# bschrag620/PyRad

Measured on NVIDIA B200. Metric: line-gridpoint evals/s, higher is better.
Workload: dtype f32

## Files before the change

### pyrad_b200/csrc/k2_line_sum.cuh

```cuda
#pragma once
#include "common.cuh"
#include "k3_stream.cuh"

namespace prb {

__device__ __forceinline__ float rcp_approx(float x) {
    float r;
    asm("rcp.approx.ftz.f32 %0, %1;" : "=f"(r) : "f"(x));
    return r;
}
__device__ __forceinline__ float ex2_approx(float x) {
    float r;
    asm("ex2.approx.ftz.f32 %0, %1;" : "=f"(r) : "f"(x));
    return r;
}

__device__ __forceinline__ void tma_bulk_s2g(void *dst, const void *src, uint32_t bytes) {
    asm volatile("cp.async.bulk.global.shared::cta.bulk_group [%0], [%1], %2;" ::"l"(dst), "r"(smem_u32(src)), "r"(bytes)
                 : "memory");
}
__device__ __forceinline__ void consumer_barrier() {
    asm volatile("bar.sync 1, %0;" ::"n"(K2_CONSUMERS * 32) : "memory");
}

__device__ __forceinline__ int warp_lower_bound(const int32_t *__restrict__ idx, int lo, int hi, long long key) {
    const int lane = threadIdx.x & 31;
    while (hi > lo) {
        const int span = hi - lo;
        const int step = (span + 31) >> 5;
        int pos = lo + (lane + 1) * step - 1;
        pos = pos < hi - 1 ? pos : hi - 1;
        const bool less = (long long)__ldg(idx + pos) < key;
        const unsigned m = __ballot_sync(0xffffffffu, less);
        const int c = __popc(m);
        int nlo = lo, nhi = hi;
        if (c > 0) { int p = lo + c * step - 1; p = p < hi - 1 ? p : hi - 1; nlo = p + 1; }
        if (c < 32) { int p = lo + (c + 1) * step - 1; p = p < hi - 1 ? p : hi - 1; nhi = p; }
        lo = nlo;
        hi = nhi;
    }
    return lo;
}

constexpr int K2_MAX_XSC = 8;
struct K2Layer {
    const float4 *recA;
    const float4 *recB;
    const float *recD;
    void *out;
    double inv_scale;
    int l_begin, l_end;
    int wm;
    int pad;
    double xsc_w[K2_MAX_XSC];
};

constexpr int K2_MAX_PEERS = 8;
constexpr int K2_MAX_DST = K2_MAX_PEERS + 1;
struct K2Fuse {
    int enabled;
    int n_dst;
    float neg_depth_log2e;
    float c2_over_t, c2_over_tsurf;
    long long n_total;
    double x0, dx, x_last;
    float *rad[K2_MAX_DST];
    float *trans[K2_MAX_DST];
};

struct K2Args {
    const K2Layer *layers;
    int n_layers;
    const int32_t *idx;
    long long i_begin;
    int n_chunk;
    int n_tiles;
    int tile_base;
    const int2 *tile_bounds;
    int variant;
    int out_mode;
    DevState *st;
    K2Fuse fuse;
    const double *far_lag;
    float far_delta[16];
    const double *far_lag2;
    float far_delta2[16];
    const double *xsc_sigma;
    long long xsc_ld;
    int n_xsc;
    int parts;
    double *part_sums;
    unsigned int *part_count;
};

__device__ __forceinline__ double k2_add_xsc(const K2Args &a, const K2Layer *L, int i, double v) {
    for (int t = 0; t < a.n_xsc; ++t)
        v = __dadd_rn(v, __dmul_rn(__ldg(a.xsc_sigma + (long long)t * a.xsc_ld + i), __ldg(&L->xsc_w[t])));
    return v;
}

constexpr int K2_FAR_NODES = 16;
constexpr int K2_FAR_RADIUS_SPANS = 1;
constexpr int K2_FAR_SUBGROUPS = 64 / K2_FAR_NODES;
constexpr int K2_FAR_FLUSH = 16;
#ifndef PRB_K2_FAR2_SPANS
#define PRB_K2_FAR2_SPANS 8
#endif
constexpr int K2_FAR2_SPANS = PRB_K2_FAR2_SPANS;
#ifndef PRB_K2_FAR2_ENABLE
#define PRB_K2_FAR2_ENABLE 1
#endif
constexpr bool K2_FAR2 = PRB_K2_FAR2_ENABLE != 0;
constexpr int K2_FAR2_MIN_DOMAINS = 4;
static_assert(K2_CONSUMERS % K2_FAR2_SPANS == 0, "a tile is a whole number of level-2 domains");

struct K2Desc {
    int tile0;
    int cnt;
    int flags;
    int layer;
    int part;
};
constexpr int K2_FIRST = 1, K2_LAST = 2, K2_END = 4;

struct K2Smem {
    float4 rA[K2_STAGES][K2_CHUNK];
    float4 rB[K2_STAGES][K2_CHUNK];
    float rD[K2_STAGES][K2_CHUNK];
    K2Desc desc[K2_STAGES];
    uint64_t full[K2_STAGES];
    uint64_t empty[K2_STAGES];
    double far2[2][K2_CONSUMERS][K2_FAR_NODES];
    double2 faracc[2][K2_CONSUMERS * 32];
    int part_last;
};

template <int P>
__host__ __device__ constexpr size_t K2_SMEM_BASE() {
    return ((sizeof(K2Smem) + (PRB_K2_ACC_SMEM ? sizeof(double) * P * K2_CONSUMERS * 32 : 0)) + 127) & ~size_t(127);
}
template <int P>
__host__ __device__ constexpr size_t K2_SMEM_BYTES(bool peer_staging) {
    return K2_SMEM_BASE<P>() + (peer_staging ? sizeof(float) * 2 * K2_CONSUMERS * 32 * P : 0);
}

template <int H>
struct Acc {
    float2 fi[H];
    float2 a32[H];
#if PRB_K2_ACC_SMEM
    double *a64;
    __device__ __forceinline__ double &acc(int p) { return a64[p * (K2_CONSUMERS * 32)]; }
#else
    double a64[2 * H];
    __device__ __forceinline__ double &acc(int p) { return a64[p]; }
#endif
    __device__ __forceinline__ void flush() {
#pragma unroll
        for (int j = 0; j < H; ++j) {
            acc(2 * j) += (double)a32[j].x;
            acc(2 * j + 1) += (double)a32[j].y;
            a32[j] = make_float2(0.f, 0.f);
        }
    }
};

__device__ __forceinline__ float2 splat(float v) { return make_float2(v, v); }
__device__ __forceinline__ float2 lo2(const float4 &v) { return make_float2(v.x, v.y); }
__device__ __forceinline__ float2 hi2(const float4 &v) { return make_float2(v.z, v.w); }

template <int H, bool MASKED>
__device__ __forceinline__ void triple_step(const float4 &a1, const float4 &a2, const float4 &a3, const float2 &B1,
                                            const float2 &B2, const float2 &B3, float wmf, Acc<H> &s) {
    const float2 nf1 = lo2(a1), nf2 = lo2(a2), nf3 = lo2(a3);
#pragma unroll
    for (int h = 0; h < H; ++h) {
        const float2 e1 = __fadd2_rn(s.fi[h], nf1);
        const float2 e2 = __fadd2_rn(s.fi[h], nf2);
        const float2 e3 = __fadd2_rn(s.fi[h], nf3);
        const float2 q1 = __ffma2_rn(e1, e1, B1);
        const float2 q2 = __ffma2_rn(e2, e2, B2);
        const float2 q3 = __ffma2_rn(e3, e3, B3);
        float2 A1 = hi2(a1), A2 = hi2(a2), A3 = hi2(a3);
        if (MASKED) {
            A1.x = fabsf(e1.x) <= wmf ? A1.x : 0.f;
            A1.y = fabsf(e1.y) <= wmf ? A1.y : 0.f;
            A2.x = fabsf(e2.x) <= wmf ? A2.x : 0.f;
            A2.y = fabsf(e2.y) <= wmf ? A2.y : 0.f;
            A3.x = fabsf(e3.x) <= wmf ? A3.x : 0.f;
            A3.y = fabsf(e3.y) <= wmf ? A3.y : 0.f;
        }
        const float2 p23 = __fmul2_rn(q2, q3);
        const float2 t = __ffma2_rn(A3, q2, __fmul2_rn(A2, q3));
        const float2 num = __ffma2_rn(q1, t, __fmul2_rn(A1, p23));
        const float2 den = __fmul2_rn(q1, p23);
        const float2 r = make_float2(rcp_approx(den.x), rcp_approx(den.y));
        s.a32[h] = __ffma2_rn(num, r, s.a32[h]);
    }
}

__device__ __forceinline__ float2 ldB(const float4 *sB, int j) { return *reinterpret_cast<const float2 *>(sB + j); }

template <int H, bool MASKED>
__device__ __forceinline__ void lorentz_paired(const float4 *sA, const float4 *sB, int js, int je, float wmf,
                                               Acc<H> &s) {
    const int n = je - js;
    if (n <= 0) return;
    int j = js;
    const int n6 = (n / 6) * 6;
    const int jq = js + n6;
    if (n6) {
        float4 xa1 = sA[j], xa2 = sA[j + 1], xa3 = sA[j + 2], ya1 = sA[j + 3], ya2 = sA[j + 4], ya3 = sA[j + 5];
        float2 xb1 = ldB(sB, j), xb2 = ldB(sB, j + 1), xb3 = ldB(sB, j + 2);
        float2 yb1 = ldB(sB, j + 3), yb2 = ldB(sB, j + 4), yb3 = ldB(sB, j + 5);
        int since = 0;
        for (j += 6; j < jq; j += 6) {
            triple_step<H, MASKED>(xa1, xa2, xa3, xb1, xb2, xb3, wmf, s);
            xa1 = sA[j]; xa2 = sA[j + 1]; xa3 = sA[j + 2];
            xb1 = ldB(sB, j); xb2 = ldB(sB, j + 1); xb3 = ldB(sB, j + 2);
            triple_step<H, MASKED>(ya1, ya2, ya3, yb1, yb2, yb3, wmf, s);
            ya1 = sA[j + 3]; ya2 = sA[j + 4]; ya3 = sA[j + 5];
            yb1 = ldB(sB, j + 3); yb2 = ldB(sB, j + 4); yb3 = ldB(sB, j + 5);
            if (++since == K2_FLUSH / 6) { s.flush(); since = 0; }
        }
        triple_step<H, MASKED>(xa1, xa2, xa3, xb1, xb2, xb3, wmf, s);
        triple_step<H, MASKED>(ya1, ya2, ya3, yb1, yb2, yb3, wmf, s);
    }
    for (j = jq; j < je; j += 3) {
        const float4 a1 = sA[j];
        const float2 B1 = ldB(sB, j);
        const float4 z = make_float4(a1.x, a1.y, 0.f, 0.f);
        const bool h2 = j + 1 < je, h3 = j + 2 < je;
        triple_step<H, MASKED>(a1, h2 ? sA[j + 1] : z, h3 ? sA[j + 2] : z, B1, h2 ? ldB(sB, j + 1) : B1,
                               h3 ? ldB(sB, j + 2) : B1, wmf, s);
    }
    s.flush();
}

#ifndef PRB_K2_GAUSS_PAIR_H
#define PRB_K2_GAUSS_PAIR_H 2
#endif
constexpr int K2_GAUSS_PAIR_H = PRB_K2_GAUSS_PAIR_H;

template <int H, bool MASKED>
__device__ __forceinline__ void gauss_pass(const float4 *sA, const float4 *sB, const float *sD, int js, int je,
                                           float wbf, float we1f, float wmf, Acc<H> &s) {
    int since = 0;
    for (int jb = js; jb < je; jb += 32) {
        const int jt = jb + (int)(threadIdx.x & 31);
        bool hit = false;
        if (jt < je) {
            const float dg = sD[jt];
            const float f = -sA[jt].x;
            hit = (dg >= 0.f) && (f + dg >= wbf) && (f - dg <= we1f);
        }
        unsigned int m = __ballot_sync(0xffffffffu, hit);
        auto one = [&](const float4 &b, float nf1) {
            const float2 nf = splat(nf1), C2 = splat(b.w);
#pragma unroll
            for (int h = 0; h < H; ++h) {
                const float2 e = __fadd2_rn(s.fi[h], nf);
                const float2 arg = __fmul2_rn(C2, __fmul2_rn(e, e));
                float2 g = splat(b.z);
                if (MASKED) {
                    g.x = fabsf(e.x) <= wmf ? b.z : 0.f;
                    g.y = fabsf(e.y) <= wmf ? b.z : 0.f;
                }
                s.a32[h] = __ffma2_rn(g, make_float2(ex2_approx(arg.x), ex2_approx(arg.y)), s.a32[h]);
            }
        };
        while (m) {
            const int j = jb + __ffs(m) - 1;
            m &= m - 1;
            if (H <= K2_GAUSS_PAIR_H && m) {
                const int j2 = jb + __ffs(m) - 1;
                m &= m - 1;
                const float4 b1 = sB[j], b2 = sB[j2];
                const float n1 = sA[j].x, n2 = sA[j2].x;
                const float2 nfa = splat(n1), nfb = splat(n2), Ca = splat(b1.w), Cb = splat(b2.w);
                float2 ta[H], tb[H], ga[H], gb[H];
#pragma unroll
                for (int h = 0; h < H; ++h) {
                    const float2 ea = __fadd2_rn(s.fi[h], nfa), eb = __fadd2_rn(s.fi[h], nfb);
                    const float2 xa = __fmul2_rn(Ca, __fmul2_rn(ea, ea)), xb = __fmul2_rn(Cb, __fmul2_rn(eb, eb));
                    ga[h] = splat(b1.z);
                    gb[h] = splat(b2.z);
                    if (MASKED) {
                        ga[h].x = fabsf(ea.x) <= wmf ? b1.z : 0.f;
                        ga[h].y = fabsf(ea.y) <= wmf ? b1.z : 0.f;
                        gb[h].x = fabsf(eb.x) <= wmf ? b2.z : 0.f;
                        gb[h].y = fabsf(eb.y) <= wmf ? b2.z : 0.f;
                    }
                    ta[h] = make_float2(ex2_approx(xa.x), ex2_approx(xa.y));
                    tb[h] = make_float2(ex2_approx(xb.x), ex2_approx(xb.y));
                }
#pragma unroll
                for (int h = 0; h < H; ++h) s.a32[h] = __ffma2_rn(gb[h], tb[h], __ffma2_rn(ga[h], ta[h], s.a32[h]));
                since += 2;
                if (since >= K2_FLUSH) { s.flush(); since = 0; }
                continue;
            }
            one(sB[j], sA[j].x);
            if (++since >= K2_FLUSH) { s.flush(); since = 0; }
        }
    }
    if (since) s.flush();
}

struct FarAcc {
    double v0, v1;
};
__device__ __forceinline__ float2 far_triple(const float4 &a1, const float4 &a2, const float4 &a3, const float2 &B1,
                                             const float2 &B2, const float2 &B3, const float2 &A1, const float2 &A2,
                                             const float2 &A3, const float2 &wb2, const float2 &del, const float2 &part) {
    const float2 e1 = __fadd2_rn(__fadd2_rn(wb2, lo2(a1)), del);
    const float2 e2 = __fadd2_rn(__fadd2_rn(wb2, lo2(a2)), del);
    const float2 e3 = __fadd2_rn(__fadd2_rn(wb2, lo2(a3)), del);
    const float2 q1 = __ffma2_rn(e1, e1, B1);
    const float2 q2 = __ffma2_rn(e2, e2, B2);
    const float2 q3 = __ffma2_rn(e3, e3, B3);
    const float2 p23 = __fmul2_rn(q2, q3);
    const float2 t = __ffma2_rn(A3, q2, __fmul2_rn(A2, q3));
    const float2 num = __ffma2_rn(q1, t, __fmul2_rn(A1, p23));
    const float2 den = __fmul2_rn(q1, p23);
    const float2 r = make_float2(rcp_approx(den.x), rcp_approx(den.y));
    return __ffma2_rn(num, r, part);
}
template <int G>
__device__ __forceinline__ void far_pass(const float4 *sA, const float4 *sB, int js, int je, float wbf, float2 del,
                                         double2 *acc, int sub) {
    const int n = je - js;
    if (n <= 0) return;
    const double2 acc0 = *acc;
    FarAcc fa{acc0.x, acc0.y};
    const float2 wb2 = splat(wbf);
    const float2 zero = make_float2(0.f, 0.f);
    int full = n / (3 * G);
    const float4 *pa = sA + js + sub;
    const float4 *pb = sB + js + sub;
    while (full > 0) {
        const int m = min(full, K2_FAR_FLUSH);
        float2 part = zero;
#pragma unroll 2
        for (int i = 0; i < m; ++i) {
            const float4 a1 = pa[0], a2 = pa[G], a3 = pa[2 * G];
            const float2 B1 = ldB(pb, 0), B2 = ldB(pb, G), B3 = ldB(pb, 2 * G);
            part = far_triple(a1, a2, a3, B1, B2, B3, hi2(a1), hi2(a2), hi2(a3), wb2, del, part);
            pa += 3 * G;
            pb += 3 * G;
        }
        fa.v0 += (double)part.x;
        fa.v1 += (double)part.y;
        full -= m;
    }
    const int j0 = js + (n / (3 * G)) * (3 * G);
    if (j0 < je) {
        const int j1 = j0 + sub, j2 = j1 + G, j3 = j1 + 2 * G;
        const int k1 = min(j1, je - 1), k2 = min(j2, je - 1), k3 = min(j3, je - 1);
        const float4 a1 = sA[k1], a2 = sA[k2], a3 = sA[k3];
        const float2 A1 = j1 < je ? hi2(a1) : zero, A2 = j2 < je ? hi2(a2) : zero, A3 = j3 < je ? hi2(a3) : zero;
        const float2 part = far_triple(a1, a2, a3, ldB(sB, k1), ldB(sB, k2), ldB(sB, k3), A1, A2, A3, wb2, del, zero);
        fa.v0 += (double)part.x;
        fa.v1 += (double)part.y;
    }
    *acc = make_double2(fa.v0, fa.v1);
}

template <int H>
__device__ __forceinline__ void general_all(const float4 *sA, const float4 *sB, int cnt, float wmf, Acc<H> &s) {
    for (int jb = 0; jb < cnt; jb += K2_FLUSH) {
        const int jend = min(jb + K2_FLUSH, cnt);
        for (int j = jb; j < jend; ++j) {
            const float4 a = sA[j], b = sB[j];
#pragma unroll
            for (int h = 0; h < H; ++h) {
                const float ex = s.fi[h].x + a.x, ey = s.fi[h].y + a.x;
                const float e2x = ex * ex, e2y = ey * ey;
                float tx = a.z * rcp_approx(e2x + b.x), ty = a.z * rcp_approx(e2y + b.x);
                tx = fmaf(b.z, ex2_approx(b.w * e2x), tx);
                ty = fmaf(b.z, ex2_approx(b.w * e2y), ty);
                s.a32[h].x += (fabsf(ex) <= wmf) ? tx : 0.f;
                s.a32[h].y += (fabsf(ey) <= wmf) ? ty : 0.f;
            }
        }
        s.flush();
    }
}

template <int P, bool FAR, bool SPLIT>
__device__ __forceinline__ void k2_line_sum_body(const K2Args &a) {
    static_assert(P >= 2 && P % 2 == 0, "points per thread must be even (packed FP32x2)");
    static_assert(!FAR || P == 4 || P == 8, "far-field tables exist for 128- and 256-point spans");
    constexpr int H = P / 2;
    constexpr int TILE = K2_CONSUMERS * 32 * P;
    constexpr int SPAN = 32 * P;
    extern __shared__ __align__(128) unsigned char smem_raw[];
    K2Smem &sm = *reinterpret_cast<K2Smem *>(smem_raw);
    const int tid = threadIdx.x, lane = tid & 31, warp = tid >> 5;

    if (tid == 0) {
        for (int s = 0; s < K2_STAGES; ++s) {
            mbar_init(&sm.full[s], 1);
            mbar_init(&sm.empty[s], K2_CONSUMERS);
        }
        asm volatile("fence.mbarrier_init.release.cluster;" ::: "memory");
        asm volatile("fence.proxy.async.shared::cta;" ::: "memory");
    }
    __syncthreads();

    if (warp == K2_CONSUMERS) {
        uint32_t it = 0;
        auto slot_acquire = [&](uint32_t &stage) {
            stage = it % K2_STAGES;
            mbar_wait_parked(&sm.empty[stage], ((it / K2_STAGES) & 1) ^ 1);
        };
        const int parts = (SPLIT && a.parts > 1) ? a.parts : 1;
        const int n_items = a.n_layers * a.n_tiles * parts;
        while (true) {
            int item = 0;
            if (lane == 0) item = (int)atomicAdd(&a.st->tile_counter, 1u);
            item = __shfl_sync(0xffffffffu, item, 0);
            if (item >= n_items) break;
            const int n_lt = a.n_layers * a.n_tiles;
            const int pidx = item / n_lt;
            const int lt = item - pidx * n_lt;
            const int half = parts >> 1, step = pidx >> 2, r = pidx & 3;
            const int part = parts < 4 ? pidx : (r == 0 ? half - 1 - step : r == 1 ? half + step : r == 2 ? step : parts - 1 - step);
            const int layer = lt / a.n_tiles;
            const int tile = a.tile_base + lt - layer * a.n_tiles;
            const K2Layer *L = a.layers + layer;
            const int wm = __ldg(&L->wm), l_begin = __ldg(&L->l_begin), l_end = __ldg(&L->l_end);
            const float4 *recA = L->recA;
            const float4 *recB = L->recB;
            const float *recD = L->recD;
            const int tile0 = tile * TILE;
            const long long k_lo = a.i_begin + tile0 - wm;
            const long long k_hi = a.i_begin + tile0 + TILE - 1 + wm + 1;
            int lo = warp_lower_bound(a.idx, l_begin, l_end, k_lo);
            const int hi = warp_lower_bound(a.idx, lo, l_end, k_hi);
            lo &= ~3;
            const int nch = hi > lo ? (hi - lo + K2_CHUNK - 1) / K2_CHUNK : 1;
            const int c0 = (int)((long long)part * nch / parts), c1 = (int)((long long)(part + 1) * nch / parts);
            const int cn = c1 > c0 ? c1 - c0 : 1;
            for (int k = 0; k < cn; ++k, ++it) {
                const int c = c0 + k;
                uint32_t stage;
                slot_acquire(stage);
                if (lane == 0) {
                    const int first = lo + c * K2_CHUNK;
                    const int cnt = c1 > c0 ? max(min(K2_CHUNK, hi - first), 0) : 0;
                    sm.desc[stage] = K2Desc{tile0, cnt, (k == 0 ? K2_FIRST : 0) | (k == cn - 1 ? K2_LAST : 0), layer, part};
                    if (cnt > 0) {
                        const uint32_t ce = (uint32_t)((cnt + 3) & ~3);
                        mbar_expect_tx(&sm.full[stage], ce * 36u);
                        tma_bulk_g2s(sm.rA[stage], recA + first, ce * 16u, &sm.full[stage]);
                        tma_bulk_g2s(sm.rB[stage], recB + first, ce * 16u, &sm.full[stage]);
                        tma_bulk_g2s(sm.rD[stage], recD + first, ce * 4u, &sm.full[stage]);
                    } else {
                        mbar_arrive(&sm.full[stage]);
                    }
                }
                __syncwarp();
            }
        }
        uint32_t stage;
        slot_acquire(stage);
        if (lane == 0) {
            sm.desc[stage] = K2Desc{0, 0, K2_END, 0, 0};
            mbar_arrive(&sm.full[stage]);
        }
        return;
    }

    float wmf = 0.f;
    Acc<H> s;
#pragma unroll
    for (int h = 0; h < H; ++h) { s.a32[h] = make_float2(0.f, 0.f); s.fi[h] = make_float2(0.f, 0.f); }
#if PRB_K2_ACC_SMEM
    s.a64 = reinterpret_cast<double *>(smem_raw + sizeof(K2Smem)) + tid;
#endif
#pragma unroll
    for (int p = 0; p < P; ++p) s.acc(p) = 0.0;
    int wb = 0;
    float wbf = 0.f, we1f = 0.f;
    double2 *far = &sm.faracc[0][tid];
    double2 *far2 = &sm.faracc[1][tid];
    float dbf = 0.f;
    uint32_t tile_par = 0;
    bool use2 = false;

    for (uint32_t it = 0;; ++it) {
        const uint32_t stage = it % K2_STAGES;
        mbar_wait(&sm.full[stage], (it / K2_STAGES) & 1);
        const K2Desc d = sm.desc[stage];
        if (d.flags & K2_END) {
            if (tid == 0) asm volatile("cp.async.bulk.wait_group 0;" ::: "memory");
            break;
        }
        if (d.flags & K2_FIRST) {
            wmf = (float)__ldg(&a.layers[d.layer].wm);
            wb = d.tile0 + warp * SPAN;
            wbf = (float)wb;
            we1f = (float)(wb + SPAN - 1);
#pragma unroll
            for (int h = 0; h < H; ++h) {
                s.a32[h] = make_float2(0.f, 0.f);
                s.fi[h] = make_float2((float)(wb + lane + 64 * h), (float)(wb + lane + 64 * h + 32));
            }
#pragma unroll
            for (int p = 0; p < P; ++p) s.acc(p) = 0.0;
            if (FAR) {
                *far = make_double2(0.0, 0.0);
                *far2 = make_double2(0.0, 0.0);
            }
            dbf = (float)(d.tile0 + (warp / K2_FAR2_SPANS) * (K2_FAR2_SPANS * SPAN));
            use2 = FAR && K2_FAR2 && wmf >= (float)(K2_FAR2_MIN_DOMAINS * K2_FAR2_SPANS * SPAN);
        }
        const int cnt = d.cnt;
        const float4 *sA = sm.rA[stage];
        const float4 *sB = sm.rB[stage];
        const float *sD = sm.rD[stage];

        if (a.variant == 0) {
            general_all<H>(sA, sB, cnt, wmf, s);
        } else if (cnt > 0) {
            float dgl = 0.f;
            for (int j = lane; j < cnt; j += 32) dgl = fmaxf(dgl, sD[j]);
            const float dgmax = __uint_as_float(__reduce_max_sync(0xffffffffu, __float_as_uint(dgl)));
            const float t0 = wbf - wmf;
            const float t5 = we1f + 1.f + wmf;
            float t1 = we1f - wmf, t4 = wbf + wmf + 1.f;
            if (t1 >= t4) { t1 = t5; t4 = t5; }
            const float g0 = fmaxf(wbf - dgmax, t0);
            const float g1 = fminf(we1f + 1.f + dgmax, t5);
            const float tfl = wbf + (float)((SPAN - 1) / 2 - K2_FAR_RADIUS_SPANS * SPAN);
            const float tfr = wbf + (float)(SPAN / 2 + K2_FAR_RADIUS_SPANS * SPAN);
            int b1, b4, bg0, bg1;
            if (FAR) {
                static_assert(K2_CHUNK <= 1024, "one level-1 sample per lane");
                const float f1 = -sA[min(32 * lane + 31, cnt - 1)].x;
                const bool v1 = 32 * lane < cnt;
                auto below = [&](float t) -> int {
                    const int nb = __popc(__ballot_sync(0xffffffffu, v1 && f1 < t));
                    const int j2 = 32 * nb + lane;
                    const bool l2 = j2 < cnt && -sA[min(j2, cnt - 1)].x < t;
                    return min(32 * nb, cnt) + __popc(__ballot_sync(0xffffffffu, l2));
                };
                constexpr int S2 = K2_FAR2_SPANS * SPAN;
                const int kp = lane & (K2_FAR_NODES / 2 - 1);
                const int sub = lane / (K2_FAR_NODES / 2);
                const float2 del = make_float2(a.far_delta[2 * kp], a.far_delta[2 * kp + 1]);
                const float2 del2 = make_float2(a.far_delta2[2 * kp], a.far_delta2[2 * kp + 1]);
                const int sub2 = (warp % K2_FAR2_SPANS) * K2_FAR_SUBGROUPS + sub;
                const float u1 = dbf + (float)(S2 - 1) - wmf, u4 = dbf + wmf + 1.f;
                const bool l2on = use2 && u1 < u4;
                b1 = below(t1);
                lorentz_paired<H, true>(sA, sB, below(t0), b1, wmf, s);
                b4 = below(t4);
                const int bfl = min(max(below(tfl), b1), b4);
                if (l2on) {
                    const int c4 = below(u4);
                    const int c1 = min(below(u1), c4);
                    const int cfl = min(max(below(dbf + (float)((S2 - 1) / 2 - K2_FAR_RADIUS_SPANS * S2)), c1), c4);
                    const int l1a = min(max(c1, b1), bfl), l1b = min(max(cfl, l1a), bfl);
                    far_pass<K2_FAR_SUBGROUPS>(sA, sB, b1, l1a, wbf, del, far, sub);
                    far_pass<K2_FAR2_SPANS * K2_FAR_SUBGROUPS>(sA, sB, c1, cfl, dbf, del2, far2, sub2);
                    far_pass<K2_FAR_SUBGROUPS>(sA, sB, l1b, bfl, wbf, del, far, sub);
                } else {
                    far_pass<K2_FAR_SUBGROUPS>(sA, sB, b1, bfl, wbf, del, far, sub);
                }
                const int bfr = min(max(below(tfr + 1.f), bfl), b4);
                lorentz_paired<H, false>(sA, sB, bfl, bfr, wmf, s);
                if (l2on) {
                    const int c4 = below(u4);
                    const int c1 = min(below(u1), c4);
                    const int cfl = min(max(below(dbf + (float)((S2 - 1) / 2 - K2_FAR_RADIUS_SPANS * S2)), c1), c4);
                    const int cfr = min(max(below(dbf + (float)(S2 / 2 + K2_FAR_RADIUS_SPANS * S2) + 1.f), cfl), c4);
                    const int r1a = min(max(cfr, bfr), b4), r1b = min(max(c4, r1a), b4);
                    far_pass<K2_FAR_SUBGROUPS>(sA, sB, bfr, r1a, wbf, del, far, sub);
                    far_pass<K2_FAR2_SPANS * K2_FAR_SUBGROUPS>(sA, sB, cfr, c4, dbf, del2, far2, sub2);
                    far_pass<K2_FAR_SUBGROUPS>(sA, sB, r1b, b4, wbf, del, far, sub);
                } else {
                    far_pass<K2_FAR_SUBGROUPS>(sA, sB, bfr, b4, wbf, del, far, sub);
                }
                lorentz_paired<H, true>(sA, sB, b4, below(t5), wmf, s);
                bg0 = below(g0);
                bg1 = below(g1);
            } else {
                int c0 = 0, c1 = 0, c4 = 0, c5 = 0, cg0 = 0, cg1 = 0;
                for (int j = lane; j < cnt; j += 32) {
                    const float f = -sA[j].x;
                    c0 += f < t0; c1 += f < t1; c4 += f < t4; c5 += f < t5; cg0 += f < g0; cg1 += f < g1;
                }
                const int b0 = __reduce_add_sync(0xffffffffu, c0);
                b1 = __reduce_add_sync(0xffffffffu, c1);
                b4 = __reduce_add_sync(0xffffffffu, c4);
                const int b5 = __reduce_add_sync(0xffffffffu, c5);
                bg0 = __reduce_add_sync(0xffffffffu, cg0);
                bg1 = __reduce_add_sync(0xffffffffu, cg1);
                lorentz_paired<H, true>(sA, sB, b0, b1, wmf, s);
                lorentz_paired<H, false>(sA, sB, b1, b4, wmf, s);
                lorentz_paired<H, true>(sA, sB, b4, b5, wmf, s);
            }
            if (dgmax > 0.f) {
                gauss_pass<H, true>(sA, sB, sD, bg0, min(bg1, b1), wbf, we1f, wmf, s);
                gauss_pass<H, false>(sA, sB, sD, max(bg0, b1), min(bg1, b4), wbf, we1f, wmf, s);
                gauss_pass<H, true>(sA, sB, sD, max(bg0, b4), bg1, wbf, we1f, wmf, s);
            }
        }
        __syncwarp();
        if (lane == 0) mbar_arrive(&sm.empty[stage]);

        if (d.flags & K2_LAST) {
            const K2Layer *L = a.layers + d.layer;
            const double inv_scale = __ldg(&L->inv_scale);
            void *out = L->out;
            const bool bulk = a.fuse.enabled && a.fuse.n_dst > 1 && d.tile0 + TILE <= a.n_chunk;
            float *stage_rad = reinterpret_cast<float *>(smem_raw + K2_SMEM_BASE<P>());
            float *stage_tr = stage_rad + TILE;
            if (bulk) {
                if (tid == 0) asm volatile("cp.async.bulk.wait_group.read 0;" ::: "memory");
                consumer_barrier();
            }
            if (FAR) {
                double v0 = far->x, v1 = far->y, w0 = far2->x, w1 = far2->y;
#pragma unroll
                for (int o = K2_FAR_NODES / 2; o < 32; o <<= 1) {
                    v0 += __shfl_xor_sync(0xffffffffu, v0, o);
                    v1 += __shfl_xor_sync(0xffffffffu, v1, o);
                    w0 += __shfl_xor_sync(0xffffffffu, w0, o);
                    w1 += __shfl_xor_sync(0xffffffffu, w1, o);
                }
                if (use2 && lane < K2_FAR_NODES / 2) {
                    sm.far2[tile_par][warp][2 * lane] = w0;
                    sm.far2[tile_par][warp][2 * lane + 1] = w1;
                }
                if (use2) consumer_barrier();
                double dn = 0.0;
                if (use2 && lane < K2_FAR_NODES) {
                    const int wd = (warp / K2_FAR2_SPANS) * K2_FAR2_SPANS;
#pragma unroll
                    for (int q = 0; q < K2_FAR2_SPANS; ++q) dn += sm.far2[tile_par][wd + q][lane];
                }
                if (use2) tile_par ^= 1u;
                constexpr int S2 = K2_FAR2_SPANS * SPAN;
                const double *lw2base = a.far_lag2 + (warp % K2_FAR2_SPANS) * SPAN + lane;
#pragma unroll 2
                for (int k = 0; k < K2_FAR_NODES; ++k) {
                    const double fk = __shfl_sync(0xffffffffu, (k & 1) ? v1 : v0, k >> 1);
                    const double *lw = a.far_lag + k * SPAN + lane;
#pragma unroll
                    for (int p = 0; p < P; ++p) s.acc(p) = fma(fk, __ldg(lw + 32 * p), s.acc(p));
                    if (use2) {
                        const double gk = __shfl_sync(0xffffffffu, dn, k);
                        const double *lw2 = lw2base + k * S2;
#pragma unroll
                        for (int p = 0; p < P; ++p) s.acc(p) = fma(gk, __ldg(lw2 + 32 * p), s.acc(p));
                    }
                }
            }
            bool finish = true;
            if (SPLIT && a.parts > 1) {
                const int lt = d.layer * a.n_tiles + (d.tile0 / TILE - a.tile_base);
                double *mine = a.part_sums + ((size_t)lt * a.parts + d.part) * TILE + warp * SPAN + lane;
#pragma unroll
                for (int p = 0; p < P; ++p) __stcg(mine + 32 * p, s.acc(p));
                __threadfence();
                consumer_barrier();
                if (tid == 0) sm.part_last = atomicAdd(a.part_count + lt, 1u) == (unsigned int)(a.parts - 1);
                consumer_barrier();
                finish = sm.part_last != 0;
                if (finish) {
                    __threadfence();
                    const double *all = a.part_sums + (size_t)lt * a.parts * TILE + warp * SPAN + lane;
#pragma unroll
                    for (int p = 0; p < P; ++p) {
                        double v = 0.0;
                        for (int q = 0; q < a.parts; ++q) v += __ldcg(all + (size_t)q * TILE + 32 * p);
                        s.acc(p) = v;
                    }
                }
            }
            if (finish) {
#pragma unroll
                for (int p = 0; p < P; ++p) {
                    const int i = wb + 32 * p + lane;
                    if (i < a.n_chunk) {
                        const double v = k2_add_xsc(a, L, i, s.acc(p) * inv_scale);
                        if (a.out_mode == 0) reinterpret_cast<double *>(out)[i] = v;
                        else reinterpret_cast<float *>(out)[i] = (float)v;
                        if (a.fuse.enabled) {
                            const double x = axis_value(a.i_begin + i, a.fuse.n_total, a.fuse.x0, a.fuse.dx, a.fuse.x_last);
                            const float nu = (float)x;
                            const float a3 = (float)(2E8 * hPlanck * (cLight * cLight) * (x * x * x));
                            const float e = (float)v * a.fuse.neg_depth_log2e;
                            const float b = planck_f32(a3, a.fuse.c2_over_t * nu);
                            const float rad = k3_fold_step(planck_f32(a3, a.fuse.c2_over_tsurf * nu), e, b);
                            const float tr = exp2f(0.f + e);
                            if (bulk) {
                                stage_rad[i - d.tile0] = rad;
                                stage_tr[i - d.tile0] = tr;
                            } else {
#pragma unroll 1
                                for (int dst = 0; dst < a.fuse.n_dst; ++dst) {
                                    a.fuse.rad[dst][i] = rad;
                                    a.fuse.trans[dst][i] = tr;
                                }
                            }
                        }
                    }
                }
                if (bulk) {
                    asm volatile("fence.proxy.async.shared::cta;" ::: "memory");
                    consumer_barrier();
                    if (tid == 0) {
#pragma unroll 1
                        for (int dst = 0; dst < a.fuse.n_dst; ++dst) {
                            tma_bulk_s2g(a.fuse.rad[dst] + d.tile0, stage_rad, TILE * 4u);
                            tma_bulk_s2g(a.fuse.trans[dst] + d.tile0, stage_tr, TILE * 4u);
                        }
                        asm volatile("cp.async.bulk.commit_group;" ::: "memory");
                    }
                }
            }
        }
    }
}

template <int P, bool SPLIT = false>
__global__ void __launch_bounds__(K2_THREADS, K2_MIN_CTAS) k2_line_sum(const K2Args a) {
    k2_line_sum_body<P, false, SPLIT>(a);
}
template <int P, bool SPLIT = false>
__global__ void __launch_bounds__(K2_THREADS, K2_MIN_CTAS) k2_line_sum_far(const K2Args a) {
    k2_line_sum_body<P, true, SPLIT>(a);
}

}
```

Measured before the change: 4954 billion.

## Interleave Gaussian-core line evaluations into the unmasked Lorentz loop via hit lists

In the non-far path, the kernel first compacts the indices of Gaussian lines that hit the window into a per-warp 16-bit list in shared memory. The list reuses the faracc area through a union, so shared memory does not grow. The unmasked Lorentz six-line loop then evaluates one Gaussian line per iteration, so the ex2 work overlaps with the rcp/FMA Lorentz work. Hits that don't fit are finished afterwards by gauss_rest and a fallback gauss_pass over the unscanned range. The cost is an extra ballot scan and a shared-memory write, plus extra register pressure in the hot loop.

```diff
diff --git a/pyrad_b200/csrc/k2_line_sum.cuh b/pyrad_b200/csrc/k2_line_sum.cuh
--- a/pyrad_b200/csrc/k2_line_sum.cuh
+++ b/pyrad_b200/csrc/k2_line_sum.cuh
@@ -123,6 +123,8 @@
 };
 constexpr int K2_FIRST = 1, K2_LAST = 2, K2_END = 4;
 
+constexpr int K2_HIT_CAP = 512;
+
 struct K2Smem {
     float4 rA[K2_STAGES][K2_CHUNK];
     float4 rB[K2_STAGES][K2_CHUNK];
@@ -131,9 +133,15 @@
     uint64_t full[K2_STAGES];
     uint64_t empty[K2_STAGES];
     double far2[2][K2_CONSUMERS][K2_FAR_NODES];
-    double2 faracc[2][K2_CONSUMERS * 32];
+    union {
+        double2 faracc[2][K2_CONSUMERS * 32];
+        uint16_t hits[K2_CONSUMERS][K2_HIT_CAP];
+    };
     int part_last;
 };
+static_assert(sizeof(uint16_t) * K2_CONSUMERS * K2_HIT_CAP <= sizeof(double2) * 2 * K2_CONSUMERS * 32,
+              "the hit lists do not grow the shared memory of the kernel");
+static_assert(K2_CHUNK <= 65536, "slot-local line indices fit 16 bits");
 
 template <int P>
 __host__ __device__ constexpr size_t K2_SMEM_BASE() {
@@ -202,8 +210,30 @@
 __device__ __forceinline__ float2 ldB(const float4 *sB, int j) { return *reinterpret_cast<const float2 *>(sB + j); }
 
 template <int H, bool MASKED>
+__device__ __forceinline__ void gauss_line(float G, float C, float nf1, float wmf, Acc<H> &s) {
+    const float2 nf = splat(nf1), C2 = splat(C);
+#pragma unroll
+    for (int h = 0; h < H; ++h) {
+        const float2 e = __fadd2_rn(s.fi[h], nf);
+        const float2 arg = __fmul2_rn(C2, __fmul2_rn(e, e));
+        float2 g = splat(G);
+        if (MASKED) {
+            g.x = fabsf(e.x) <= wmf ? G : 0.f;
+            g.y = fabsf(e.y) <= wmf ? G : 0.f;
+        }
+        s.a32[h] = __ffma2_rn(g, make_float2(ex2_approx(arg.x), ex2_approx(arg.y)), s.a32[h]);
+    }
+}
+
+struct GaussHits {
+    const uint16_t *list;
+    int next, n;
+};
+
+template <int H, bool MASKED, bool GAUSS = false>
 __device__ __forceinline__ void lorentz_paired(const float4 *sA, const float4 *sB, int js, int je, float wmf,
-                                               Acc<H> &s) {
+                                               Acc<H> &s, GaussHits *gh = nullptr) {
+    static_assert(!(MASKED && GAUSS), "Gaussian cores ride along with full-cover lines only");
     const int n = je - js;
     if (n <= 0) return;
     int j = js;
@@ -214,15 +244,31 @@
         float2 xb1 = ldB(sB, j), xb2 = ldB(sB, j + 1), xb3 = ldB(sB, j + 2);
         float2 yb1 = ldB(sB, j + 3), yb2 = ldB(sB, j + 4), yb3 = ldB(sB, j + 5);
         int since = 0;
-        for (j += 6; j < jq; j += 6) {
+        const int mix = GAUSS ? min(gh->n - gh->next, n6 / 6 - 1) : 0;
+        const uint16_t *hit = GAUSS ? gh->list + gh->next : nullptr;
+        auto six = [&](auto with_gauss) {
+            float2 GC;
+            float gnf;
+            if (decltype(with_gauss)::value) {
+                const int jh = *hit++;
+                GC = reinterpret_cast<const float2 *>(sB + jh)[1];
+                gnf = sA[jh].x;
+            }
             triple_step<H, MASKED>(xa1, xa2, xa3, xb1, xb2, xb3, wmf, s);
+            if (decltype(with_gauss)::value)
+                gauss_line<H, false>(GC.x, GC.y, gnf, wmf, s);
             xa1 = sA[j]; xa2 = sA[j + 1]; xa3 = sA[j + 2];
             xb1 = ldB(sB, j); xb2 = ldB(sB, j + 1); xb3 = ldB(sB, j + 2);
             triple_step<H, MASKED>(ya1, ya2, ya3, yb1, yb2, yb3, wmf, s);
             ya1 = sA[j + 3]; ya2 = sA[j + 4]; ya3 = sA[j + 5];
             yb1 = ldB(sB, j + 3); yb2 = ldB(sB, j + 4); yb3 = ldB(sB, j + 5);
             if (++since == K2_FLUSH / 6) { s.flush(); since = 0; }
-        }
+            j += 6;
+        };
+        j += 6;
+        for (int k = 0; k < mix; ++k) six(std::true_type{});
+        if (GAUSS) gh->next += mix;
+        while (j < jq) six(std::false_type{});
         triple_step<H, MASKED>(xa1, xa2, xa3, xb1, xb2, xb3, wmf, s);
         triple_step<H, MASKED>(ya1, ya2, ya3, yb1, yb2, yb3, wmf, s);
     }
@@ -255,20 +301,6 @@
             hit = (dg >= 0.f) && (f + dg >= wbf) && (f - dg <= we1f);
         }
         unsigned int m = __ballot_sync(0xffffffffu, hit);
-        auto one = [&](const float4 &b, float nf1) {
-            const float2 nf = splat(nf1), C2 = splat(b.w);
-#pragma unroll
-            for (int h = 0; h < H; ++h) {
-                const float2 e = __fadd2_rn(s.fi[h], nf);
-                const float2 arg = __fmul2_rn(C2, __fmul2_rn(e, e));
-                float2 g = splat(b.z);
-                if (MASKED) {
-                    g.x = fabsf(e.x) <= wmf ? b.z : 0.f;
-                    g.y = fabsf(e.y) <= wmf ? b.z : 0.f;
-                }
-                s.a32[h] = __ffma2_rn(g, make_float2(ex2_approx(arg.x), ex2_approx(arg.y)), s.a32[h]);
-            }
-        };
         while (m) {
             const int j = jb + __ffs(m) - 1;
             m &= m - 1;
@@ -300,9 +332,43 @@
                 if (since >= K2_FLUSH) { s.flush(); since = 0; }
                 continue;
             }
-            one(sB[j], sA[j].x);
+            const float4 b = sB[j];
+            gauss_line<H, MASKED>(b.z, b.w, sA[j].x, wmf, s);
             if (++since >= K2_FLUSH) { s.flush(); since = 0; }
         }
+    }
+    if (since) s.flush();
+}
+
+__device__ __forceinline__ int gauss_hits(const float4 *sA, const float *sD, int js, int je, float wbf, float we1f,
+                                          uint16_t *list, GaussHits &gh) {
+    const int lane = threadIdx.x & 31;
+    int n = 0, jb = js;
+    for (; jb < je && n <= K2_HIT_CAP - 32; jb += 32) {
+        const int jt = jb + lane;
+        bool hit = false;
+        if (jt < je) {
+            const float dg = sD[jt];
+            const float f = -sA[jt].x;
+            hit = (dg >= 0.f) && (f + dg >= wbf) && (f - dg <= we1f);
+        }
+        const unsigned int m = __ballot_sync(0xffffffffu, hit);
+        if (hit) list[n + __popc(m & ((1u << lane) - 1u))] = (uint16_t)jt;
+        n += __popc(m);
+    }
+    __syncwarp();
+    gh = GaussHits{list, 0, n};
+    return jb < je ? jb : je;
+}
+
+template <int H>
+__device__ __forceinline__ void gauss_rest(const float4 *sA, const float4 *sB, const GaussHits &gh, float wmf, Acc<H> &s) {
+    int since = 0;
+    for (int k = gh.next; k < gh.n; ++k) {
+        const int j = gh.list[k];
+        const float4 b = sB[j];
+        gauss_line<H, false>(b.z, b.w, sA[j].x, wmf, s);
+        if (++since >= K2_FLUSH) { s.flush(); since = 0; }
     }
     if (since) s.flush();
 }
@@ -586,6 +652,11 @@
                 lorentz_paired<H, true>(sA, sB, b4, below(t5), wmf, s);
                 bg0 = below(g0);
                 bg1 = below(g1);
+                if (dgmax > 0.f) {
+                    gauss_pass<H, true>(sA, sB, sD, bg0, min(bg1, b1), wbf, we1f, wmf, s);
+                    gauss_pass<H, false>(sA, sB, sD, max(bg0, b1), min(bg1, b4), wbf, we1f, wmf, s);
+                    gauss_pass<H, true>(sA, sB, sD, max(bg0, b4), bg1, wbf, we1f, wmf, s);
+                }
             } else {
                 int c0 = 0, c1 = 0, c4 = 0, c5 = 0, cg0 = 0, cg1 = 0;
                 for (int j = lane; j < cnt; j += 32) {
@@ -598,14 +669,19 @@
                 const int b5 = __reduce_add_sync(0xffffffffu, c5);
                 bg0 = __reduce_add_sync(0xffffffffu, cg0);
                 bg1 = __reduce_add_sync(0xffffffffu, cg1);
+                GaussHits gh{nullptr, 0, 0};
+                const int gf0 = max(bg0, b1), gf1 = min(bg1, b4);
+                int gr = gf1;
+                if (dgmax > 0.f) gr = gauss_hits(sA, sD, gf0, gf1, wbf, we1f, sm.hits[warp], gh);
                 lorentz_paired<H, true>(sA, sB, b0, b1, wmf, s);
-                lorentz_paired<H, false>(sA, sB, b1, b4, wmf, s);
+                lorentz_paired<H, false, true>(sA, sB, b1, b4, wmf, s, &gh);
                 lorentz_paired<H, true>(sA, sB, b4, b5, wmf, s);
-            }
-            if (dgmax > 0.f) {
-                gauss_pass<H, true>(sA, sB, sD, bg0, min(bg1, b1), wbf, we1f, wmf, s);
-                gauss_pass<H, false>(sA, sB, sD, max(bg0, b1), min(bg1, b4), wbf, we1f, wmf, s);
-                gauss_pass<H, true>(sA, sB, sD, max(bg0, b4), bg1, wbf, we1f, wmf, s);
+                if (dgmax > 0.f) {
+                    gauss_rest<H>(sA, sB, gh, wmf, s);
+                    gauss_pass<H, false>(sA, sB, sD, gr, gf1, wbf, we1f, wmf, s);
+                    gauss_pass<H, true>(sA, sB, sD, bg0, min(bg1, b1), wbf, we1f, wmf, s);
+                    gauss_pass<H, true>(sA, sB, sD, max(bg0, b4), bg1, wbf, we1f, wmf, s);
+                }
             }
         }
         __syncwarp();
```

Result: faster. 5079 billion, median of 6 (+2.5%).
